# sandyz1000/deep-insight-face

Measured on AMD Instinct MI355X. Metric: faces/sec embedding+match (112x112, 512-d), higher is better.
Workload: dtype f32; 1 GPU; configs[3]: IResNet-100 embed, batch=512/GPU (4096 on 8 GPUs), 1M gallery row-sharded; arch=iresnet100, head=v2, batch_per_gpu=512, global_batch=512, gallery_rows=1000000, gallery_rows_per_gpu=1000000, emd=512, metric=cosine, parallelism=dp1 + gallery row-shard

## Files before the change

### deep-insight-face_amd/csrc/conv_winograd.hpp

```cpp
namespace wino {
constexpr int BN = 64;
constexpr int KC = 16;
constexpr int64_t MIN_TILES = 64 * 49;
constexpr int WIDE_MAX_HW = 112;
constexpr int64_t WIDE_MIN_IMAGES = 128;
constexpr int ODD_MAX_HW = 16;
constexpr int64_t ODD_MIN_TILES = 128 * 16;
}

template <int TT_, int CPW_, int MIN_BLOCKS_, bool EARLY_REQ_>
struct WinoW {
  static constexpr int TT = TT_;
  static constexpr int CPW = CPW_;
  static constexpr int MIN_BLOCKS = MIN_BLOCKS_;
  static constexpr bool EARLY_REQ = EARLY_REQ_;
  static constexpr bool ODD = false;
  static constexpr bool YSUB = false;
  static constexpr int MF = TT / 32;
  static constexpr int NT = 16 / CPW * 64;
  static constexpr int STAGE = 16 * TT * wino::KC;
  static constexpr int LDS_BYTES = 2 * STAGE * 4;
  static_assert(NT / 8 == TT && CPW % 2 == 0, "one loader thread per (tile, channel pair)");
};

template <bool ODD_, bool YSUB_>
struct WinoX : WinoW<32, 4, 2, true> {
  static constexpr bool ODD = ODD_;
  static constexpr bool YSUB = YSUB_;
  static_assert(!(ODD_ && YSUB_), "y_sub is admitted on even maps only");
};

__device__ __forceinline__ void wino_bt4(float x0, float x1, float x2, float x3, float& o0, float& o1, float& o2, float& o3) {
  o0 = x0 - x2;
  o1 = x1 + x2;
  o2 = x2 - x1;
  o3 = x1 - x3;
}

__device__ __forceinline__ void wino_input_transform(const float (&d)[16], float (&v)[16]) {
  float t[16];
#pragma unroll
  for (int c = 0; c < 4; ++c) wino_bt4(d[c], d[4 + c], d[8 + c], d[12 + c], t[c], t[4 + c], t[8 + c], t[12 + c]);
#pragma unroll
  for (int r = 0; r < 4; ++r) wino_bt4(t[4 * r], t[4 * r + 1], t[4 * r + 2], t[4 * r + 3], v[4 * r], v[4 * r + 1], v[4 * r + 2], v[4 * r + 3]);
}

template <bool TRACE>
__device__ __forceinline__ unsigned long long wino_stamp() {
  if constexpr (TRACE) return __builtin_amdgcn_s_memrealtime();
  return 0ull;
}
__device__ __forceinline__ void wino_trace_write(const ConvArgs& a, unsigned long long c0, const unsigned long long (&ts)[5]) {
  unsigned long long* t = a.trace + (size_t)blockIdx.x * 8;
  t[0] = ts[2] - ts[1];
  t[1] = ts[1] - ts[0];
  t[2] = ts[3] - ts[2];
  t[3] = ts[4] - ts[3];
  t[4] = (unsigned long long)__builtin_amdgcn_s_getreg((31 << 11) | 4) | ((unsigned long long)__builtin_amdgcn_s_getreg((31 << 11) | 20) << 32);
  t[5] = ts[0];
  t[6] = ts[4];
  t[7] = 3 | ((__builtin_amdgcn_s_memtime() - c0) << 8);
}

template <class S, bool TRACE>
__global__ __launch_bounds__(S::NT, S::MIN_BLOCKS) void conv_wino_kernel(const ConvArgs a, int blocks_m, int nblocks) {
  constexpr int TT = S::TT, CPW = S::CPW, MF = S::MF, KC = wino::KC;
  extern __shared__ __attribute__((aligned(16))) float wino_smem[];
  const int b = xcd_remap((int)blockIdx.x, nblocks);
  const int nt = b / blocks_m, mt = b - nt * blocks_m;
  const int tid = threadIdx.x, lane = tid & 63;
  const int wave = (S::ODD || S::YSUB) ? __builtin_amdgcn_readfirstlane(tid >> 6) : tid >> 6;
  const int tw = S::ODD ? (a.W + 1) >> 1 : a.W >> 1, tpi = (S::ODD ? (a.H + 1) >> 1 : a.H >> 1) * tw, ntiles = a.N * tpi;
  const int KS = a.Cin / KC;
  unsigned long long ts[5];
  ts[0] = wino_stamp<TRACE>();
  const unsigned long long tr_c0 = TRACE ? __builtin_amdgcn_s_memtime() : 0ull;

  const int ltile = tid >> 3, cp = tid & 7;
  const int g = mt * TT + ltile;
  const bool tile_ok = g < ntiles;
  int pix0 = 0;
  unsigned vmask = 0;
  if (tile_ok) {
    const int img = g / tpi, rem = g - img * tpi, ty = rem / tw, tx = rem - ty * tw;
    pix0 = (img * a.H + 2 * ty) * a.W + 2 * tx;
#pragma unroll
    for (int p = 0; p < 16; ++p) {
      const int iy = 2 * ty - 1 + (p >> 2), ix = 2 * tx - 1 + (p & 3);
      if (iy >= 0 && iy < a.H && ix >= 0 && ix < a.W) vmask |= 1u << p;
    }
  }
  const int row_b = a.W * a.Cin * 4, pix_b = a.Cin * 4;
  const int lbase = (pix0 - a.W - 1) * pix_b + cp * 8;
  const __amdgpu_buffer_rsrc_t xrs = make_rsrc(a.x, (uint32_t)a.N * (uint32_t)(a.H * a.W) * (uint32_t)pix_b);
  auto dload = [&](int ks, f32x2 (&d)[16]) {
#pragma unroll
    for (int p = 0; p < 16; ++p) {
      const uint32_t off = ((vmask >> p) & 1u) ? (uint32_t)(lbase + (p >> 2) * row_b + (p & 3) * pix_b + ks * (KC * 4)) : OOB;
      d[p] = __builtin_bit_cast(f32x2, __builtin_amdgcn_raw_buffer_load_b64(xrs, off, 0, 0));
    }
  };
  const int vdst = ltile * KC + (((cp >> 1) ^ ((ltile >> 2) & 3)) << 2) + (cp & 1) * 2;
  auto vstore = [&](float* buf, const f32x2 (&d)[16]) {
    float d0[16], d1[16], v0[16], v1[16];
#pragma unroll
    for (int p = 0; p < 16; ++p) {
      d0[p] = d[p][0];
      d1[p] = d[p][1];
    }
    wino_input_transform(d0, v0);
    wino_input_transform(d1, v1);
#pragma unroll
    for (int c = 0; c < 16; ++c) *reinterpret_cast<f32x2*>(buf + c * (TT * KC) + vdst) = f32x2{v0[c], v1[c]};
  };

  const int h = lane >> 5, r32 = lane & 31, sw = (r32 >> 2) & 3;
  const int tiles_n = a.Cout / wino::BN;
  const __amdgpu_buffer_rsrc_t wrs = make_rsrc(a.w_wino, a.w_wino_bytes);
  const uint32_t boff0 = (uint32_t)((CPW * wave * tiles_n + nt) * KS) * 4096u + (uint32_t)lane * 16u;
  const uint32_t bstep = (uint32_t)(tiles_n * KS) * 4096u;
  f32x4 bw[2][2][2];
  auto bload = [&](int j, int ks) {
#pragma unroll
    for (int nf = 0; nf < 2; ++nf)
#pragma unroll
      for (int q = 0; q < 2; ++q)
        bw[j & 1][nf][q] = buf_load4(wrs, boff0 + (uint32_t)j * bstep + (uint32_t)ks * 4096u + (uint32_t)(nf * 2 + q) * 1024u);
  };
  int aoff[2];
#pragma unroll
  for (int q = 0; q < 2; ++q) aoff[q] = r32 * KC + (((2 * h + q) ^ sw) << 2);
  f32x4 av[2][MF][2];
  auto aread = [&](const float* buf, int j) {
#pragma unroll
    for (int mf = 0; mf < MF; ++mf)
#pragma unroll
      for (int q = 0; q < 2; ++q)
        av[j & 1][mf][q] = *reinterpret_cast<const f32x4*>(buf + (CPW * wave + j) * (TT * KC) + mf * 32 * KC + aoff[q]);
  };
  f32x16 acc[CPW][MF][2];
#pragma unroll
  for (int j = 0; j < CPW; ++j)
#pragma unroll
    for (int mf = 0; mf < MF; ++mf)
#pragma unroll
      for (int nf = 0; nf < 2; ++nf)
#pragma unroll
        for (int r = 0; r < 16; ++r) acc[j][mf][nf][r] = 0.f;
  auto mfma = [&](int j) {
#pragma unroll
    for (int q = 0; q < 2; ++q)
#pragma unroll
      for (int t = 0; t < 4; ++t)
#pragma unroll
        for (int mf = 0; mf < MF; ++mf)
#pragma unroll
          for (int nf = 0; nf < 2; ++nf)
            acc[j][mf][nf] = __builtin_amdgcn_mfma_f32_32x32x2f32(av[j & 1][mf][q][t], bw[j & 1][nf][q][t], acc[j][mf][nf], 0, 0, 0);
  };

  {
    f32x2 d[16];
    dload(0, d);
    bload(0, 0);
    bload(1, 0);
    vstore(wino_smem, d);
    lds_barrier();
    ts[1] = wino_stamp<TRACE>();
    auto step = [&](int ks, auto last) {
      const float* cur = wino_smem + (ks & 1) * S::STAGE;
      float* nxt = wino_smem + ((ks + 1) & 1) * S::STAGE;
      aread(cur, 0);
      aread(cur, 1);
#pragma unroll
      for (int j = 0; j < CPW; ++j) {
        mfma(j);
        __builtin_amdgcn_sched_barrier(0);
        if (j + 2 < CPW) {
          aread(cur, j + 2);
          bload(j + 2, ks);
        } else if (!last.value) {
          bload(j + 2 - CPW, ks + 1);
        }
        if (!last.value && j == CPW / 2 - 1) dload(ks + 1, d);
        __builtin_amdgcn_sched_barrier(0);
      }
      if (!last.value) vstore(nxt, d);
      lds_barrier();
    };
    for (int ks = 0; ks + 1 < KS; ++ks) step(ks, std::false_type{});
    step(KS - 1, std::true_type{});
  }
  ts[2] = wino_stamp<TRACE>();

  const int c4 = cp * 4;
  const uint32_t bytes = (uint32_t)a.M * (uint32_t)a.Cout * 4u;
  const __amdgpu_buffer_rsrc_t y_rsrc = make_rsrc(a.y, a.y ? (S::YSUB ? (uint32_t)ntiles * (uint32_t)a.Cout * 4u : bytes) : 0u);
  const __amdgpu_buffer_rsrc_t y2_rsrc = make_rsrc(a.y2, a.y2 ? bytes : 0u);
  const __amdgpu_buffer_rsrc_t res_rsrc = make_rsrc(a.res, a.res ? bytes : 0u);
  const bool has_res = a.res != nullptr;
  const int act = a.act, act2 = a.act2;
#pragma unroll
  for (int nf = 0; nf < 2; ++nf) {
    const int c = nt * wino::BN + nf * 32 + c4;
    f32x4 sc, sh, al, sc2, sh2, al2, rv[4];
    uint32_t voff[4];
    if constexpr (S::EARLY_REQ) {
      sc = load4_or(a.scale, c, 1.f), sh = load4_or(a.shift, c, 0.f), al = load4_or(a.alpha, c, 0.f);
      sc2 = load4_or(a.scale2, c, 1.f), sh2 = load4_or(a.shift2, c, 0.f), al2 = load4_or(a.alpha2, c, 0.f);
#pragma unroll
      for (int p = 0; p < 4; ++p) {
        const int pix = pix0 + (p >> 1) * a.W + (p & 1);
        if constexpr (S::ODD)
          voff[p] = ((vmask >> (5 + 4 * (p >> 1) + (p & 1))) & 1u) ? ((uint32_t)pix * (uint32_t)a.Cout + (uint32_t)c) * 4u : OOB;
        else
          voff[p] = tile_ok ? ((uint32_t)pix * (uint32_t)a.Cout + (uint32_t)c) * 4u : OOB;
        rv[p] = has_res ? buf_load4(res_rsrc, voff[p]) : f32x4{0.f, 0.f, 0.f, 0.f};
      }
      __builtin_amdgcn_sched_barrier(0);
    }
#pragma unroll
    for (int j = 0; j < CPW; ++j)
#pragma unroll
      for (int mf = 0; mf < MF; ++mf)
#pragma unroll
        for (int r = 0; r < 16; ++r)
          wino_smem[(CPW * wave + j) * (TT * 32) + (mf * 32 + frag_row(lane, r)) * 32 + r32] = acc[j][mf][nf][r];
    lds_barrier();
    f32x4 m[16];
#pragma unroll
    for (int k = 0; k < 16; ++k) m[k] = *reinterpret_cast<const f32x4*>(wino_smem + k * (TT * 32) + ltile * 32 + c4);
    f32x4 yv[4];
    {
      f32x4 s0[4], s1[4];
#pragma unroll
      for (int jj = 0; jj < 4; ++jj) {
        s0[jj] = m[jj] + m[4 + jj] + m[8 + jj];
        s1[jj] = m[4 + jj] - m[8 + jj] - m[12 + jj];
      }
      yv[0] = s0[0] + s0[1] + s0[2];
      yv[1] = s0[1] - s0[2] - s0[3];
      yv[2] = s1[0] + s1[1] + s1[2];
      yv[3] = s1[1] - s1[2] - s1[3];
    }
    if constexpr (!S::EARLY_REQ) {
      sc = load4_or(a.scale, c, 1.f), sh = load4_or(a.shift, c, 0.f), al = load4_or(a.alpha, c, 0.f);
      sc2 = load4_or(a.scale2, c, 1.f), sh2 = load4_or(a.shift2, c, 0.f), al2 = load4_or(a.alpha2, c, 0.f);
#pragma unroll
      for (int p = 0; p < 4; ++p) {
        const int pix = pix0 + (p >> 1) * a.W + (p & 1);
        if constexpr (S::ODD)
          voff[p] = ((vmask >> (5 + 4 * (p >> 1) + (p & 1))) & 1u) ? ((uint32_t)pix * (uint32_t)a.Cout + (uint32_t)c) * 4u : OOB;
        else
          voff[p] = tile_ok ? ((uint32_t)pix * (uint32_t)a.Cout + (uint32_t)c) * 4u : OOB;
        rv[p] = has_res ? buf_load4(res_rsrc, voff[p]) : f32x4{0.f, 0.f, 0.f, 0.f};
      }
    }
#pragma unroll
    for (int p = 0; p < 4; ++p) {
      f32x4 v, v2;
      epilogue4(yv[p], sc, sh, al, act, has_res, rv[p], sc2, sh2, al2, act2, v, v2);
      if constexpr (S::YSUB) {
        if (p == 0) __builtin_amdgcn_raw_buffer_store_b128(__builtin_bit_cast(u32x4, v), y_rsrc, tile_ok ? ((uint32_t)g * (uint32_t)a.Cout + (uint32_t)c) * 4u : OOB, 0, 0);
      } else {
        __builtin_amdgcn_raw_buffer_store_b128(__builtin_bit_cast(u32x4, v), y_rsrc, voff[p], 0, 0);
      }
      __builtin_amdgcn_raw_buffer_store_b128(__builtin_bit_cast(u32x4, v2), y2_rsrc, voff[p], 0, 0);
    }
    lds_barrier();
    ts[3 + nf] = wino_stamp<TRACE>();
  }
  if constexpr (TRACE)
    if (tid == 0) wino_trace_write(a, tr_c0, ts);
}

static int wino_applies(const ConvArgs& a) {
  if (!a.w_wino || a.wino_level < 1 || a.KH != 3 || a.KW != 3 || a.stride != 1 || a.pad_t != 1 || a.pad_l != 1) return 0;
  if (a.Ho != a.H || a.Wo != a.W) return 0;
  const bool odd = (a.H & 1) || (a.W & 1), rest = odd || a.y_sub;
  const bool wide = a.H > 16 || a.W > 16;
  if (rest && (a.wino_level < 2 || (odd && (a.y_sub || a.H > wino::ODD_MAX_HW || a.W > wino::ODD_MAX_HW || a.H < 3 || a.W < 3)))) return 0;
  if (wide && (a.wino_level < 2 || a.H > wino::WIDE_MAX_HW || a.W > wino::WIDE_MAX_HW)) return 0;
  if (a.Cin % 32 != 0 || a.Cout % wino::BN != 0 || a.pre_scale) return 0;
  if (!(a.y_H == a.Ho && a.y_W == a.Wo && a.y_oy == 0 && a.y_ox == 0 && a.y_ld == a.Cout && a.y_coff == 0)) return 0;
  if (a.res && (a.res_stride != 1 || a.res_H != a.Ho || a.res_W != a.Wo)) return 0;
  if ((int64_t)a.M * a.Cout * 4 >= 0x7fffffffLL || (int64_t)a.M * a.Cin * 4 >= 0x7fffffffLL) return 0;
  if ((int64_t)16 * a.Cin * a.Cout * 4 > (int64_t)a.w_wino_bytes) return 0;
  const int64_t tpi = (int64_t)((a.H + 1) / 2) * ((a.W + 1) / 2);
  if (rest) return a.N >= wino::WIDE_MIN_IMAGES && (!odd || a.N * tpi >= wino::ODD_MIN_TILES) ? 3 : 0;
  if (wide) return a.N * tpi >= wino::WIDE_MIN_IMAGES * tpi ? 2 : 0;
  return a.N * tpi >= wino::MIN_TILES ? 1 : 0;
}

template <class S>
static int launch_wino(const ConvArgs& a, hipStream_t st, const char* name) {
  const auto kern = a.trace ? conv_wino_kernel<S, true> : conv_wino_kernel<S, false>;
  if (allow_dynamic_lds(reinterpret_cast<const void*>(kern), S::LDS_BYTES)) return -1;
  const int64_t ntiles = S::ODD ? (int64_t)a.N * ((a.H + 1) / 2) * ((a.W + 1) / 2) : (int64_t)a.N * (a.H / 2) * (a.W / 2);
  const int blocks_m = (int)((ntiles + S::TT - 1) / S::TT), tiles_n = a.Cout / wino::BN;
  const int64_t nblocks = (int64_t)blocks_m * tiles_n;
  if (nblocks >= 0x7fffffffLL) return set_error("conv: too many tiles");
  hipLaunchKernelGGL(kern, dim3((unsigned)nblocks), dim3(S::NT), S::LDS_BYTES, st, a, blocks_m, (int)nblocks);
  DIF_HIP(hipGetLastError());
  g_last_kernel = name;
  return 0;
}

static int launch_conv_wino(const ConvArgs& a, hipStream_t st) {
  if (a.wino_level >= 2 && !(a.dbg & 16777216)) return launch_wino<WinoW<32, 4, 2, true>>(a, st, "conv_wino_kernel<F(2x2,3x3),32 tiles x 64>");
  return launch_wino<WinoW<64, 2, 1, false>>(a, st, "conv_wino_kernel<F(2x2,3x3),64 tiles x 64>");
}

static int launch_conv_winow(const ConvArgs& a, hipStream_t st) {
  if (a.dbg & 65536) return launch_wino<WinoW<64, 2, 2, true>>(a, st, "conv_winow_kernel<F(2x2,3x3),64 tiles x 64>");
  return launch_wino<WinoW<32, 4, 2, true>>(a, st, "conv_winow_kernel<F(2x2,3x3),32 tiles x 64>");
}

static int launch_conv_winox(const ConvArgs& a, hipStream_t st) {
  if (a.y_sub) return launch_wino<WinoX<false, true>>(a, st, "conv_winox_kernel<F(2x2,3x3),32 tiles x 64,ysub>");
  return launch_wino<WinoX<true, false>>(a, st, "conv_winox_kernel<F(2x2,3x3),32 tiles x 64,odd>");
}
```

### deep-insight-face_amd/csrc/net.hip

```cpp
#include "net.hpp"

#include <math.h>
#include <stdio.h>
#include <stdlib.h>
#include <string.h>

#include <algorithm>
#include <map>

#include "../../include/dif.h"
#include "dif_internal.hpp"
#include "gemm_core.hpp"

namespace dif {

static const float EPS_RESNET = 1.001e-5f;
static const float EPS_KERAS = 1e-3f;
static const float EPS_IRESNET = 1e-5f;

Net::~Net() { release_device(); }

void Net::release_device() {
  for (Lane& L : lanes) {
    if (L.stream) (void)hipStreamDestroy(L.stream);
// ... 1266 lines not shown
      a.pad_l = op.pad_l;
      a.Kpad = op.Kpad;
      a.k_order = op.k_order;
      a.M = n * yd.H * yd.W;
      a.act = op.act;
      a.act2 = op.act2;
      a.y_sub = op.y_sub;
      if (op.res >= 0) {
        a.res_H = tensors[op.res].H;
        a.res_W = tensors[op.res].W;
        a.res_stride = op.res_stride;
      } else {
        a.res_H = yd.H;
        a.res_W = yd.W;
        a.res_stride = 1;
      }
      {
        const TensorDesc& vd = tensors[op.y >= 0 ? op.y : op.y2];
        if (vd.parent >= 0) {
          const TensorDesc& pd = tensors[vd.parent];
          a.y_ld = pd.C;
          a.y_coff = vd.coff;
          a.y_H = pd.H;
          a.y_W = pd.W;
          a.y_oy = vd.oy;
          a.y_ox = vd.ox;
        } else {
          a.y_ld = op.Cout;
          a.y_coff = 0;
          a.y_H = yd.H;
          a.y_W = yd.W;
          a.y_oy = a.y_ox = 0;
        }
      }
      a.sk_slab = L.sk_slab;
      a.sk_flag = L.sk_flag;
      a.sk_max_blocks = lanes_active ? L.sk_max_blocks : sk_max_blocks;
      a.sk_epoch = ++L.sk_epoch;
      a.sk_spin_limit = sk_spin_limit;
      a.use_pipe = use_pipe;
      a.off = conv_off;
      a.dbg = conv_dbg;
      a.lanes = lanes_active ? (int)lanes.size() : 1;
      a.bdp_mode = use_bdp == 2 ? 2 : ((use_bdp == 0 || lane_split) ? 1 : 0);
      a.trace = trace_buf ? trace_buf + trace_off[&op - ops.data()] * 8 : nullptr;
      if (op.d_w_raw && op.stem_mfma && use_stem) {
        if (stem_mfma_run(a.x, op.d_w_raw, a.scale, a.shift, a.alpha, a.scale2, a.shift2, a.alpha2, a.y, a.y2, n, a.H, a.W,
                          a.Ho, a.Wo, a.KH, a.stride, a.act, a.act2, a.y_sub, st))
          return -1;
        break;
      }
      if (op.d_w_raw && use_stem) {
        if (stem3x3_run(a.x, op.d_w_raw, a.scale, a.shift, a.alpha, a.scale2, a.shift2, a.alpha2, a.y, a.y2, n, a.H, a.W, a.Cout,
                        a.act, a.act2, st))
          return -1;
        break;
      }
      if (conv_run(a, st)) return -1;
      op.ran_kernel = conv_last_kernel();
      break;
    }
    case OP_MAXPOOL: {
      const TensorDesc& xd = tensors[op.x];
      const TensorDesc& yd = tensors[op.y];
      PoolArgs a;
      memset(&a, 0, sizeof(a));
      a.x = ptr(op.x);
      a.y = ptr(op.y);
      a.y2 = ptr(op.y2);
      a.scale2 = op.d_scale2;
      a.shift2 = op.d_shift2;
      a.N = n;
      a.H = xd.H;
      a.W = xd.W;
      a.C = xd.C;
      a.Ho = yd.H;
      a.Wo = yd.W;
      a.k = op.KH;
      a.stride = op.stride;
      a.pad_t = op.pad_t;
      a.pad_l = op.pad_l;
      a.zero_pad = op.zero_pad;
      a.act2 = op.act2;
      a.mode = op.pool_mode;
      if (yd.parent >= 0) {
        const TensorDesc& pd = tensors[yd.parent];
        a.y_ld = pd.C;
        a.y_coff = yd.coff;
        a.y_H = pd.H;
        a.y_W = pd.W;
        a.y_oy = yd.oy;
        a.y_ox = yd.ox;
      } else {
        a.y_ld = yd.C;
        a.y_coff = 0;
        a.y_H = yd.H;
        a.y_W = yd.W;
        a.y_oy = a.y_ox = 0;
      }
      if (maxpool_run(a, st)) return -1;
      break;
    }
    case OP_GDCTAIL: {
      const TensorDesc& xd = tensors[op.x];
      if (gdc_tail_run(ptr(op.x), op.d_w, op.d_scale, op.d_shift, op.d_w_pw, op.d_w_dense, ptr(op.y), n, xd.H * xd.W,
                       op.Cout, 1e-12f, L.tail_ws, st))
        return -1;
      op.ran_kernel = n <= 2 && op.Cout % 32 == 0 ? "gdc_tail_a_kernel+gdc_tail_b_kernel" : "gdc_tail_kernel";
      break;
    }
    case OP_DWFULL: {
      const TensorDesc& xd = tensors[op.x];
      if (dwfull_run(ptr(op.x), op.d_w, op.d_scale, op.d_shift, ptr(op.y), n, xd.H * xd.W, xd.C, st)) return -1;
      break;
    }
    case OP_DWCONV: {
      const TensorDesc& xd = tensors[op.x];
      const TensorDesc& yd = tensors[op.y];
      if (dwconv_run(ptr(op.x), op.d_w, op.d_scale, op.d_shift, ptr(op.y), n, xd.H, xd.W, xd.C, op.KH, op.stride, op.pad_t,
                     op.pad_l, yd.H, yd.W, op.act, st))
        return -1;
      break;
    }
    case OP_LRN: {
      const TensorDesc& xd = tensors[op.x];
      if (lrn_run(ptr(op.x), ptr(op.y), (int64_t)n * xd.H * xd.W, xd.C, 5, 1.f, 1e-4f, 0.75f, st)) return -1;
      break;
    }
    case OP_UPSAMPLE: {
      const TensorDesc& xd = tensors[op.x];
      const TensorDesc& yd = tensors[op.y];
      const int ld = yd.parent >= 0 ? tensors[yd.parent].C : yd.C;
      if (upsample2_run(ptr(op.x), ptr(op.y), n, xd.H, xd.W, xd.C, ld, yd.coff, st)) return -1;
      break;
    }
    case OP_COPY: {
      const TensorDesc& xd = tensors[op.x];
      const TensorDesc& yd = tensors[op.y];
      const int ld = yd.parent >= 0 ? tensors[yd.parent].C : yd.C;
      if (copy_to_view_run(ptr(op.x), ptr(op.y), (int64_t)n * xd.H * xd.W, xd.C, ld, yd.coff, st)) return -1;
      break;
    }
    case OP_ZERO: {
      const TensorDesc& yd = tensors[op.y];
      DIF_HIP(hipMemsetAsync(ptr(op.y), 0, (size_t)n * yd.elems() * sizeof(float), st));
      break;
    }
    case OP_L2NORM:
      if (l2norm_run(ptr(op.x), ptr(op.y), n, op.Cout, 1e-12f, st)) return -1;
      break;
  }
  return 0;
}

int Net::embed(const void* xin, int n, int layout, int dtype, float* out, hipStream_t st, float* op_ms) {
  if (!finalized) return set_error("dif_net_embed: call dif_net_finalize first");
  if (n < 0 || n > max_batch) return set_error("dif_net_embed: batch %d outside [0, max_batch=%d]", n, max_batch);
  if (n == 0) return 0;
  if (!xin || !out) return set_error("dif_net_embed: null pointer");
  if (layout != DIF_LAYOUT_NHWC && layout != DIF_LAYOUT_NCHW) return set_error("dif_net_embed: bad layout %d", layout);
  if (dtype != DIF_DTYPE_F32 && dtype != DIF_DTYPE_U8) return set_error("dif_net_embed: bad dtype %d", dtype);

  const int nl = (int)lanes.size();
  lanes_active = !(op_ms || nl == 1 || n < lane_min_images());
  lanes[0].out_n = n;
  lanes[0].out_start = 0;
  if (!lanes_active) {
    std::vector<hipEvent_t> ev;
    if (op_ms) {
      ev.resize(ops.size() + 1);
      for (auto& e : ev) DIF_HIP(hipEventCreate(&e));
      DIF_HIP(hipEventRecord(ev[0], st));
    }
    for (size_t i = 0; i < ops.size(); ++i) {
      if (run_op(ops[i], lanes[0], xin, n, layout, dtype, out, st)) return -1;
      if (op_ms) DIF_HIP(hipEventRecord(ev[i + 1], st));
    }
    if (op_ms) {
      DIF_HIP(hipStreamSynchronize(st));
      for (size_t i = 0; i < ops.size(); ++i) DIF_HIP(hipEventElapsedTime(&op_ms[i], ev[i], ev[i + 1]));
      for (auto& e : ev) (void)hipEventDestroy(e);
    }
    return 0;
  }

  const size_t in_bytes = (size_t)in_h * in_w * 3 * (dtype == DIF_DTYPE_U8 ? 1 : 4);
  std::vector<int> start(nl + 1, 0);
  for (int l = 0; l < nl; ++l) {
    int c = n / nl + (l < n % nl ? 1 : 0);
    if (l > 0 && c > lanes[l].cap) c = lanes[l].cap;
    start[l + 1] = start[l] + c;
  }
  const int l_first = lanes[0].stream ? 0 : 1;
  DIF_HIP(hipEventRecord(ev_start, st));
  for (int l = l_first; l < nl; ++l) DIF_HIP(hipStreamWaitEvent(lanes[l].stream, ev_start, 0));
  for (size_t i = 0; i < ops.size(); ++i) {
    for (int l = 0; l < nl; ++l) {
      const int c = start[l + 1] - start[l];
      if (c == 0) continue;
      hipStream_t ls = lanes[l].stream ? lanes[l].stream : st;
      lanes[l].out_n = n;
      lanes[l].out_start = start[l];
      if (run_op(ops[i], lanes[l], static_cast<const char*>(xin) + (size_t)start[l] * in_bytes, c, layout, dtype, out, ls))
        return -1;
    }
  }
  for (int l = l_first; l < nl; ++l) {
    DIF_HIP(hipEventRecord(lanes[l].done, lanes[l].stream));
    DIF_HIP(hipStreamWaitEvent(st, lanes[l].done, 0));
  }
  return 0;
}

int Net::embed_clock(const void* xin, int n, int layout, int dtype, float* out, hipStream_t st, double* ghz) {
  if (!finalized) return set_error("dif_net_embed_clock: call dif_net_finalize first");
  if (!ghz) return set_error("dif_net_embed_clock: null output");
  if (n < 1 || n > max_batch) return set_error("dif_net_embed_clock: batch %d outside [1, max_batch=%d]", n, max_batch);
  trace_off.assign(ops.size(), 0);
  size_t total = 0;
  for (size_t i = 0; i < ops.size(); ++i) {
    trace_off[i] = total;
    if (ops[i].kind != OP_CONV) continue;
    const TensorDesc& yd = tensors[ops[i].y >= 0 && !ops[i].y_sub ? ops[i].y : ops[i].y2];
    const size_t tiles = (((size_t)n * yd.H * yd.W + 63) / 64) * (((size_t)ops[i].Cout + 63) / 64);
    total += tiles > (size_t)sk_max_blocks ? tiles : (size_t)sk_max_blocks;
  }
  unsigned long long* d = nullptr;
  DIF_HIP(hipMalloc(&d, total * 8 * sizeof(unsigned long long)));
  DIF_HIP(hipMemsetAsync(d, 0, total * 8 * sizeof(unsigned long long), st));
  trace_buf = d;
  int rc = 0;
  lanes_active = false;
  lanes[0].out_n = n;
  lanes[0].out_start = 0;
  for (size_t i = 0; i < ops.size() && !rc; ++i) rc = run_op(ops[i], lanes[0], xin, n, layout, dtype, out, st);
  trace_buf = nullptr;
  std::vector<unsigned long long> h;
  if (!rc) {
    h.resize(total * 8);
    if (hipStreamSynchronize(st) != hipSuccess || hipMemcpy(h.data(), d, h.size() * sizeof(unsigned long long), hipMemcpyDeviceToHost) != hipSuccess)
      rc = set_error("dif_net_embed_clock: reading the records failed");
  }
  (void)hipFree(d);
  if (rc) return rc;
  if (conv_dbg & 256) {
    for (size_t i = 0; i < ops.size(); ++i) {
      if (ops[i].kind != OP_CONV) continue;
      const size_t end = i + 1 < ops.size() ? trace_off[i + 1] : total;
      unsigned long long t_lo = ~0ull, t_hi = 0;
      double life = 0, mn = 1e30, mx = 0, m = 0, f = 0, e = 0, steps = 0, tiles = 0;
      double p_set = 0, p_pro = 0, p_steps = 0, p_hand = 0, p_tiles = 0;
      double w_e0 = 0, w_e1 = 0;
      std::map<unsigned long long, std::vector<const unsigned long long*>> w_cu;
      int nb = 0;
      for (size_t b = trace_off[i]; b < end; ++b) {
        const unsigned long long* t = &h[b * 8];
        if ((t[7] & 0xff) == 0 || t[6] <= t[5]) continue;
        ++nb;
        t_lo = t[5] < t_lo ? t[5] : t_lo;
        t_hi = t[6] > t_hi ? t[6] : t_hi;
        const double l = (double)(t[6] - t[5]);
        life += l;
        mn = l < mn ? l : mn;
        mx = l > mx ? l : mx;
        if ((t[7] & 0xff) == 2) {
          p_set += (double)t[0];
          p_pro += (double)t[1];
          p_steps += (double)t[2];
          p_hand += (double)t[3];
          p_tiles += (double)t[4];
        }
        if ((t[7] & 0xff) == 1) {
          m += (double)t[0];
          f += (double)t[1];
          e += (double)t[2];
          steps += (double)t[3];
          tiles += (double)t[4];
        }
        if ((t[7] & 0xff) == 3) {
          m += (double)t[0];
          f += (double)t[1];
          e += (double)(t[2] + t[3]);
          w_e0 += (double)t[2];
          w_e1 += (double)t[3];
          tiles += 1;
          w_cu[((t[4] >> 32) & 0xf) << 16 | (t[4] & 0xff00)].push_back(t);
        }
      }
      if (nb)
        fprintf(stderr, "trace %-22s blocks %5d span %7.1f us | life mean %7.1f min %7.1f max %7.1f | main %6.1f fix %6.1f epi %6.1f us/block | "
                        "steps/block %.1f tiles/block %.2f\n", ops[i].name.c_str(), nb, (double)(t_hi - t_lo) / 100.0, life / nb / 100.0,
                mn / 100.0, mx / 100.0, m / nb / 100.0, f / nb / 100.0, e / nb / 100.0, steps / nb, tiles / nb);
      if (nb && !w_cu.empty()) {
        double ph = 0, lag = 0;
        int pairs = 0;
        for (auto& kv : w_cu)
          for (const unsigned long long* u : kv.second)
            for (const unsigned long long* v : kv.second)
              if (v != u && v[5] <= u[5] && u[5] < v[6] && (v[5] < u[5] || v < u)) {
                ph += (double)(u[5] - v[5]) / (double)(v[6] - v[5]);
                lag += (double)(u[5] - v[5]);
                ++pairs;
              }
        fprintf(stderr, "      winograd: epilogue halves %.1f + %.1f us/block | %zu CUs, %.2f blocks/CU | blocks starting beside a resident one: %d, "
                        "%.1f us = %.2f of its life after it\n", w_e0 / nb / 100.0, w_e1 / nb / 100.0, w_cu.size(), (double)nb / w_cu.size(), pairs,
                pairs ? lag / pairs / 100.0 : 0.0, pairs ? ph / pairs : 0.0);
      }
      if (nb && p_tiles > 0)
        fprintf(stderr, "      pipelined: %.2f tiles/block | per tile: set-up %.2f prologue %.2f K-steps %.2f hand-over %.2f us\n", p_tiles / nb,
                p_set / p_tiles / 100.0, p_pro / p_tiles / 100.0, p_steps / p_tiles / 100.0, p_hand / p_tiles / 100.0);
    }
  }
  if (conv_dbg & 512) {
    for (size_t i = 0; i < ops.size(); ++i) {
      if (ops[i].kind != OP_CONV) continue;
      const size_t end = i + 1 < ops.size() ? trace_off[i + 1] : total;
      std::map<unsigned, std::vector<double>> by_xcd, by_cu;
      unsigned long long t_lo = ~0ull;
      for (size_t b = trace_off[i]; b < end; ++b)
        if ((h[b * 8 + 7] & 0xff) == 1 && h[b * 8 + 4] && h[b * 8 + 5] < t_lo) t_lo = h[b * 8 + 5];
      int nb = 0;
      for (size_t b = trace_off[i]; b < end; ++b) {
        const unsigned long long* t = &h[b * 8];
        if ((t[7] & 0xff) != 1 || !t[4] || t[6] <= t[5]) continue;
        ++nb;
        const unsigned hw = (unsigned)t[4], xcc = (unsigned)(t[4] >> 32) & 0xf;
        const unsigned cu = (xcc << 16) | (hw & 0xff00);
        for (auto* mp : {&by_xcd[xcc], &by_cu[cu]}) {
          if (mp->empty()) mp->assign(5, 0.0);
          (*mp)[0] += 1;
          (*mp)[1] += (double)(t[6] - t[5]);
          (*mp)[2] += (double)(t[7] >> 8);
          (*mp)[3] = std::max((*mp)[3], (double)(t[6] - t_lo));
          (*mp)[4] += (double)(t[5] - t_lo);
        }
      }
      if (!nb) continue;
      fprintf(stderr, "place %-20s blocks %d on %zu CUs |", ops[i].name.c_str(), nb, by_cu.size());
      for (auto& kv : by_xcd)
        fprintf(stderr, " xcd%u: %d blk life %.0f us end %.0f us %.2f GHz |", kv.first, (int)kv.second[0], kv.second[1] / kv.second[0] / 100.0,
                kv.second[3] / 100.0, kv.second[2] / (kv.second[1] * 10.0));
      std::map<int, std::vector<double>> hist;
      for (auto& kv : by_cu) {
        auto& hrec = hist[(int)kv.second[0]];
        if (hrec.empty()) hrec.assign(4, 0.0);
        hrec[0] += 1;
        hrec[1] += kv.second[1] / kv.second[0];
        hrec[2] += kv.second[3];
        hrec[3] += kv.second[4] / kv.second[0];
      }
      for (auto& kv : hist)
        fprintf(stderr, " %d/CU: %d CUs life %.0f start %.0f end %.0f us |", kv.first, (int)kv.second[0], kv.second[1] / kv.second[0] / 100.0,
                kv.second[3] / kv.second[0] / 100.0, kv.second[2] / kv.second[0] / 100.0);
      double rl[8] = {0}, rn[8] = {0}, wl[16] = {0}, wn[16] = {0};
      for (size_t b = trace_off[i]; b < end; ++b) {
        const unsigned long long* t = &h[b * 8];
        if ((t[7] & 0xff) != 1 || !t[4] || t[6] <= t[5]) continue;
        const size_t r = std::min<size_t>((b - trace_off[i]) / by_cu.size(), 7);
        rl[r] += (double)(t[6] - t[5]);
        rn[r] += 1;
        wl[t[4] & 0xf] += (double)(t[6] - t[5]);
        wn[t[4] & 0xf] += 1;
      }
      for (int r = 0; r < 8; ++r)
        if (rn[r] > 0) fprintf(stderr, " round%d: %.0f us (%d) |", r, rl[r] / rn[r] / 100.0, (int)rn[r]);
      for (int r = 0; r < 16; ++r)
        if (wn[r] > 0) fprintf(stderr, " slot%d: %.0f us (%d) |", r, wl[r] / wn[r] / 100.0, (int)wn[r]);
      fprintf(stderr, "\n");
    }
  }
  double cyc = 0, ticks = 0;
  for (size_t b = 0; b < total; ++b) {
    const unsigned long long* t = &h[b * 8];
    const unsigned kind = (unsigned)(t[7] & 0xff);
    if ((kind == 1 || kind == 2) && t[6] > t[5]) {
      cyc += (double)(t[7] >> 8);
      ticks += (double)(t[6] - t[5]);
    }
  }
  *ghz = ticks > 0 ? cyc / (ticks * 10.0) : 0.0;
  return 0;
}

}
```

Before: 8853 faces/s.

## Fold Winograd output rows in registers and issue residual loads under last K-step

For the CPW=4 Winograd config, each wave now owns one column of the 4x4 transform grid. It performs the first stage of the output transform in registers, stages only two planes per nf to LDS, and finishes both channel halves in a single pass with one barrier. The old code staged all sixteen planes per half with two barriers. Residual loads are also issued during the final K-step so their latency hides behind MFMAs. This costs extra registers for the prefetched residuals and changes the weight and LDS indexing, which could lower occupancy.

```diff
diff --git a/deep-insight-face_amd/csrc/conv_winograd.hpp b/deep-insight-face_amd/csrc/conv_winograd.hpp
--- a/deep-insight-face_amd/csrc/conv_winograd.hpp
+++ b/deep-insight-face_amd/csrc/conv_winograd.hpp
@@ -7,6 +7,10 @@
 constexpr int ODD_MAX_HW = 16;
 constexpr int64_t ODD_MIN_TILES = 128 * 16;
 }
+
+#ifndef DIF_WINO_RES_UNDER_K
+#define DIF_WINO_RES_UNDER_K 1
+#endif
 
 template <int TT_, int CPW_, int MIN_BLOCKS_, bool EARLY_REQ_>
 struct WinoW {
@@ -20,7 +24,12 @@
   static constexpr int NT = 16 / CPW * 64;
   static constexpr int STAGE = 16 * TT * wino::KC;
   static constexpr int LDS_BYTES = 2 * STAGE * 4;
+  static constexpr bool ONE_PASS = CPW_ == 4;
+  static constexpr int COMP_W = ONE_PASS ? 1 : CPW_;
+  static constexpr int COMP_J = ONE_PASS ? 4 : 1;
+  static constexpr bool RES_UNDER_K = ONE_PASS && DIF_WINO_RES_UNDER_K;
   static_assert(NT / 8 == TT && CPW % 2 == 0, "one loader thread per (tile, channel pair)");
+  static_assert(!ONE_PASS || (TT == 32 && 8 * TT * wino::BN * 4 <= LDS_BYTES), "one pass: eight planes of 32 tiles x 64 channels");
 };
 
 template <bool ODD_, bool YSUB_>
@@ -117,8 +126,8 @@
   const int h = lane >> 5, r32 = lane & 31, sw = (r32 >> 2) & 3;
   const int tiles_n = a.Cout / wino::BN;
   const __amdgpu_buffer_rsrc_t wrs = make_rsrc(a.w_wino, a.w_wino_bytes);
-  const uint32_t boff0 = (uint32_t)((CPW * wave * tiles_n + nt) * KS) * 4096u + (uint32_t)lane * 16u;
-  const uint32_t bstep = (uint32_t)(tiles_n * KS) * 4096u;
+  const uint32_t boff0 = (uint32_t)((S::COMP_W * wave * tiles_n + nt) * KS) * 4096u + (uint32_t)lane * 16u;
+  const uint32_t bstep = (uint32_t)(S::COMP_J * tiles_n * KS) * 4096u;
   f32x4 bw[2][2][2];
   auto bload = [&](int j, int ks) {
 #pragma unroll
@@ -136,7 +145,7 @@
     for (int mf = 0; mf < MF; ++mf)
 #pragma unroll
       for (int q = 0; q < 2; ++q)
-        av[j & 1][mf][q] = *reinterpret_cast<const f32x4*>(buf + (CPW * wave + j) * (TT * KC) + mf * 32 * KC + aoff[q]);
+        av[j & 1][mf][q] = *reinterpret_cast<const f32x4*>(buf + (S::COMP_W * wave + S::COMP_J * j) * (TT * KC) + mf * 32 * KC + aoff[q]);
   };
   f32x16 acc[CPW][MF][2];
 #pragma unroll
@@ -157,6 +166,21 @@
 #pragma unroll
           for (int nf = 0; nf < 2; ++nf)
             acc[j][mf][nf] = __builtin_amdgcn_mfma_f32_32x32x2f32(av[j & 1][mf][q][t], bw[j & 1][nf][q][t], acc[j][mf][nf], 0, 0, 0);
+  };
+
+  uint32_t voff8[2][4];
+  f32x4 rv8[2][4];
+  auto res_request = [&]() {
+    const __amdgpu_buffer_rsrc_t res_rsrc = make_rsrc(a.res, a.res ? (uint32_t)a.M * (uint32_t)a.Cout * 4u : 0u);
+#pragma unroll
+    for (int nf = 0; nf < 2; ++nf)
+#pragma unroll
+      for (int p = 0; p < 4; ++p) {
+        const int pix = pix0 + (p >> 1) * a.W + (p & 1), c = nt * wino::BN + nf * 32 + cp * 4;
+        const uint32_t off_map = ((vmask >> (5 + 4 * (p >> 1) + (p & 1))) & 1u) - 1u;
+        voff8[nf][p] = (((uint32_t)pix * (uint32_t)a.Cout + (uint32_t)c) * 4u) | (off_map & OOB);
+        rv8[nf][p] = buf_load4(res_rsrc, voff8[nf][p]);
+      }
   };
 
   {
@@ -183,6 +207,7 @@
           bload(j + 2 - CPW, ks + 1);
         }
         if (!last.value && j == CPW / 2 - 1) dload(ks + 1, d);
+        if (last.value && S::RES_UNDER_K && j == CPW / 2 - 1) res_request();
         __builtin_amdgcn_sched_barrier(0);
       }
       if (!last.value) vstore(nxt, d);
@@ -200,75 +225,130 @@
   const __amdgpu_buffer_rsrc_t res_rsrc = make_rsrc(a.res, a.res ? bytes : 0u);
   const bool has_res = a.res != nullptr;
   const int act = a.act, act2 = a.act2;
-#pragma unroll
-  for (int nf = 0; nf < 2; ++nf) {
-    const int c = nt * wino::BN + nf * 32 + c4;
-    f32x4 sc, sh, al, sc2, sh2, al2, rv[4];
-    uint32_t voff[4];
-    if constexpr (S::EARLY_REQ) {
-      sc = load4_or(a.scale, c, 1.f), sh = load4_or(a.shift, c, 0.f), al = load4_or(a.alpha, c, 0.f);
-      sc2 = load4_or(a.scale2, c, 1.f), sh2 = load4_or(a.shift2, c, 0.f), al2 = load4_or(a.alpha2, c, 0.f);
-#pragma unroll
-      for (int p = 0; p < 4; ++p) {
-        const int pix = pix0 + (p >> 1) * a.W + (p & 1);
-        if constexpr (S::ODD)
-          voff[p] = ((vmask >> (5 + 4 * (p >> 1) + (p & 1))) & 1u) ? ((uint32_t)pix * (uint32_t)a.Cout + (uint32_t)c) * 4u : OOB;
-        else
-          voff[p] = tile_ok ? ((uint32_t)pix * (uint32_t)a.Cout + (uint32_t)c) * 4u : OOB;
-        rv[p] = has_res ? buf_load4(res_rsrc, voff[p]) : f32x4{0.f, 0.f, 0.f, 0.f};
-      }
-      __builtin_amdgcn_sched_barrier(0);
-    }
-#pragma unroll
-    for (int j = 0; j < CPW; ++j)
-#pragma unroll
-      for (int mf = 0; mf < MF; ++mf)
-#pragma unroll
-        for (int r = 0; r < 16; ++r)
-          wino_smem[(CPW * wave + j) * (TT * 32) + (mf * 32 + frag_row(lane, r)) * 32 + r32] = acc[j][mf][nf][r];
+  if constexpr (S::ONE_PASS) {
+    static_assert(MF == 1 && CPW == 4, "one row fragment, one grid column per wave");
+    if constexpr (!S::RES_UNDER_K) res_request();
+    f32x4 sc[2], sh[2], al[2], sc2[2], sh2[2], al2[2];
+#pragma unroll
+    for (int nf = 0; nf < 2; ++nf) {
+      const int c = nt * wino::BN + nf * 32 + c4;
+      sc[nf] = load4_or(a.scale, c, 1.f), sh[nf] = load4_or(a.shift, c, 0.f), al[nf] = load4_or(a.alpha, c, 0.f);
+      sc2[nf] = load4_or(a.scale2, c, 1.f), sh2[nf] = load4_or(a.shift2, c, 0.f), al2[nf] = load4_or(a.alpha2, c, 0.f);
+    }
+    __builtin_amdgcn_sched_barrier(0);
+#pragma unroll
+    for (int nf = 0; nf < 2; ++nf) {
+      acc[3][0][nf] = (acc[1][0][nf] - acc[2][0][nf]) - acc[3][0][nf];
+      acc[0][0][nf] = (acc[0][0][nf] + acc[1][0][nf]) + acc[2][0][nf];
+    }
+#pragma unroll
+    for (int nf = 0; nf < 2; ++nf)
+#pragma unroll
+      for (int r = 0; r < 16; ++r) {
+        wino_smem[(wave * 2 + nf) * (TT * 32) + frag_row(lane, r) * 32 + r32] = acc[0][0][nf][r];
+        wino_smem[((4 + wave) * 2 + nf) * (TT * 32) + frag_row(lane, r) * 32 + r32] = acc[3][0][nf][r];
+      }
     lds_barrier();
-    f32x4 m[16];
-#pragma unroll
-    for (int k = 0; k < 16; ++k) m[k] = *reinterpret_cast<const f32x4*>(wino_smem + k * (TT * 32) + ltile * 32 + c4);
-    f32x4 yv[4];
-    {
+    ts[3] = wino_stamp<TRACE>();
+#pragma unroll
+    for (int nf = 0; nf < 2; ++nf) {
       f32x4 s0[4], s1[4];
 #pragma unroll
       for (int jj = 0; jj < 4; ++jj) {
-        s0[jj] = m[jj] + m[4 + jj] + m[8 + jj];
-        s1[jj] = m[4 + jj] - m[8 + jj] - m[12 + jj];
-      }
+        s0[jj] = *reinterpret_cast<const f32x4*>(wino_smem + (jj * 2 + nf) * (TT * 32) + ltile * 32 + c4);
+        s1[jj] = *reinterpret_cast<const f32x4*>(wino_smem + ((4 + jj) * 2 + nf) * (TT * 32) + ltile * 32 + c4);
+      }
+      f32x4 yv[4];
       yv[0] = s0[0] + s0[1] + s0[2];
       yv[1] = s0[1] - s0[2] - s0[3];
       yv[2] = s1[0] + s1[1] + s1[2];
       yv[3] = s1[1] - s1[2] - s1[3];
-    }
-    if constexpr (!S::EARLY_REQ) {
-      sc = load4_or(a.scale, c, 1.f), sh = load4_or(a.shift, c, 0.f), al = load4_or(a.alpha, c, 0.f);
-      sc2 = load4_or(a.scale2, c, 1.f), sh2 = load4_or(a.shift2, c, 0.f), al2 = load4_or(a.alpha2, c, 0.f);
 #pragma unroll
       for (int p = 0; p < 4; ++p) {
-        const int pix = pix0 + (p >> 1) * a.W + (p & 1);
-        if constexpr (S::ODD)
-          voff[p] = ((vmask >> (5 + 4 * (p >> 1) + (p & 1))) & 1u) ? ((uint32_t)pix * (uint32_t)a.Cout + (uint32_t)c) * 4u : OOB;
-        else
-          voff[p] = tile_ok ? ((uint32_t)pix * (uint32_t)a.Cout + (uint32_t)c) * 4u : OOB;
-        rv[p] = has_res ? buf_load4(res_rsrc, voff[p]) : f32x4{0.f, 0.f, 0.f, 0.f};
-      }
-    }
-#pragma unroll
-    for (int p = 0; p < 4; ++p) {
-      f32x4 v, v2;
-      epilogue4(yv[p], sc, sh, al, act, has_res, rv[p], sc2, sh2, al2, act2, v, v2);
-      if constexpr (S::YSUB) {
-        if (p == 0) __builtin_amdgcn_raw_buffer_store_b128(__builtin_bit_cast(u32x4, v), y_rsrc, tile_ok ? ((uint32_t)g * (uint32_t)a.Cout + (uint32_t)c) * 4u : OOB, 0, 0);
-      } else {
-        __builtin_amdgcn_raw_buffer_store_b128(__builtin_bit_cast(u32x4, v), y_rsrc, voff[p], 0, 0);
-      }
-      __builtin_amdgcn_raw_buffer_store_b128(__builtin_bit_cast(u32x4, v2), y2_rsrc, voff[p], 0, 0);
-    }
-    lds_barrier();
-    ts[3 + nf] = wino_stamp<TRACE>();
+        f32x4 v, v2;
+        epilogue4(yv[p], sc[nf], sh[nf], al[nf], act, has_res, rv8[nf][p], sc2[nf], sh2[nf], al2[nf], act2, v, v2);
+        if constexpr (S::YSUB) {
+          if (p == 0)
+            __builtin_amdgcn_raw_buffer_store_b128(__builtin_bit_cast(u32x4, v), y_rsrc,
+                                                   tile_ok ? ((uint32_t)g * (uint32_t)a.Cout + (uint32_t)(nt * wino::BN + nf * 32 + c4)) * 4u : OOB, 0, 0);
+        } else {
+          __builtin_amdgcn_raw_buffer_store_b128(__builtin_bit_cast(u32x4, v), y_rsrc, voff8[nf][p], 0, 0);
+        }
+        __builtin_amdgcn_raw_buffer_store_b128(__builtin_bit_cast(u32x4, v2), y2_rsrc, voff8[nf][p], 0, 0);
+      }
+    }
+    ts[4] = wino_stamp<TRACE>();
+  } else {
+#pragma unroll
+    for (int nf = 0; nf < 2; ++nf) {
+      const int c = nt * wino::BN + nf * 32 + c4;
+      f32x4 sc, sh, al, sc2, sh2, al2, rv[4];
+      uint32_t voff[4];
+      if constexpr (S::EARLY_REQ) {
+        sc = load4_or(a.scale, c, 1.f), sh = load4_or(a.shift, c, 0.f), al = load4_or(a.alpha, c, 0.f);
+        sc2 = load4_or(a.scale2, c, 1.f), sh2 = load4_or(a.shift2, c, 0.f), al2 = load4_or(a.alpha2, c, 0.f);
+#pragma unroll
+        for (int p = 0; p < 4; ++p) {
+          const int pix = pix0 + (p >> 1) * a.W + (p & 1);
+          if constexpr (S::ODD)
+            voff[p] = ((vmask >> (5 + 4 * (p >> 1) + (p & 1))) & 1u) ? ((uint32_t)pix * (uint32_t)a.Cout + (uint32_t)c) * 4u : OOB;
+          else
+            voff[p] = tile_ok ? ((uint32_t)pix * (uint32_t)a.Cout + (uint32_t)c) * 4u : OOB;
+          rv[p] = has_res ? buf_load4(res_rsrc, voff[p]) : f32x4{0.f, 0.f, 0.f, 0.f};
+        }
+        __builtin_amdgcn_sched_barrier(0);
+      }
+#pragma unroll
+      for (int j = 0; j < CPW; ++j)
+#pragma unroll
+        for (int mf = 0; mf < MF; ++mf)
+#pragma unroll
+          for (int r = 0; r < 16; ++r)
+            wino_smem[(CPW * wave + j) * (TT * 32) + (mf * 32 + frag_row(lane, r)) * 32 + r32] = acc[j][mf][nf][r];
+      lds_barrier();
+      f32x4 m[16];
+#pragma unroll
+      for (int k = 0; k < 16; ++k) m[k] = *reinterpret_cast<const f32x4*>(wino_smem + k * (TT * 32) + ltile * 32 + c4);
+      f32x4 yv[4];
+      {
+        f32x4 s0[4], s1[4];
+#pragma unroll
+        for (int jj = 0; jj < 4; ++jj) {
+          s0[jj] = m[jj] + m[4 + jj] + m[8 + jj];
+          s1[jj] = m[4 + jj] - m[8 + jj] - m[12 + jj];
+        }
+        yv[0] = s0[0] + s0[1] + s0[2];
+        yv[1] = s0[1] - s0[2] - s0[3];
+        yv[2] = s1[0] + s1[1] + s1[2];
+        yv[3] = s1[1] - s1[2] - s1[3];
+      }
+      if constexpr (!S::EARLY_REQ) {
+        sc = load4_or(a.scale, c, 1.f), sh = load4_or(a.shift, c, 0.f), al = load4_or(a.alpha, c, 0.f);
+        sc2 = load4_or(a.scale2, c, 1.f), sh2 = load4_or(a.shift2, c, 0.f), al2 = load4_or(a.alpha2, c, 0.f);
+#pragma unroll
+        for (int p = 0; p < 4; ++p) {
+          const int pix = pix0 + (p >> 1) * a.W + (p & 1);
+          if constexpr (S::ODD)
+            voff[p] = ((vmask >> (5 + 4 * (p >> 1) + (p & 1))) & 1u) ? ((uint32_t)pix * (uint32_t)a.Cout + (uint32_t)c) * 4u : OOB;
+          else
+            voff[p] = tile_ok ? ((uint32_t)pix * (uint32_t)a.Cout + (uint32_t)c) * 4u : OOB;
+          rv[p] = has_res ? buf_load4(res_rsrc, voff[p]) : f32x4{0.f, 0.f, 0.f, 0.f};
+        }
+      }
+#pragma unroll
+      for (int p = 0; p < 4; ++p) {
+        f32x4 v, v2;
+        epilogue4(yv[p], sc, sh, al, act, has_res, rv[p], sc2, sh2, al2, act2, v, v2);
+        if constexpr (S::YSUB) {
+          if (p == 0) __builtin_amdgcn_raw_buffer_store_b128(__builtin_bit_cast(u32x4, v), y_rsrc, tile_ok ? ((uint32_t)g * (uint32_t)a.Cout + (uint32_t)c) * 4u : OOB, 0, 0);
+        } else {
+          __builtin_amdgcn_raw_buffer_store_b128(__builtin_bit_cast(u32x4, v), y_rsrc, voff[p], 0, 0);
+        }
+        __builtin_amdgcn_raw_buffer_store_b128(__builtin_bit_cast(u32x4, v2), y2_rsrc, voff[p], 0, 0);
+      }
+      lds_barrier();
+      ts[3 + nf] = wino_stamp<TRACE>();
+    }
   }
   if constexpr (TRACE)
     if (tid == 0) wino_trace_write(a, tr_c0, ts);
diff --git a/deep-insight-face_amd/csrc/net.hip b/deep-insight-face_amd/csrc/net.hip
--- a/deep-insight-face_amd/csrc/net.hip
+++ b/deep-insight-face_amd/csrc/net.hip
@@ -1592,7 +1592,7 @@
                 lag += (double)(u[5] - v[5]);
                 ++pairs;
               }
-        fprintf(stderr, "      winograd: epilogue halves %.1f + %.1f us/block | %zu CUs, %.2f blocks/CU | blocks starting beside a resident one: %d, "
+        fprintf(stderr, "      winograd: epilogue halves | stage + finish %.1f + %.1f us/block | %zu CUs, %.2f blocks/CU | blocks starting beside a resident one: %d, "
                         "%.1f us = %.2f of its life after it\n", w_e0 / nb / 100.0, w_e1 / nb / 100.0, w_cu.size(), (double)nb / w_cu.size(), pairs,
                 pairs ? lag / pairs / 100.0 : 0.0, pairs ? ph / pairs : 0.0);
       }
```

After: 8992 faces/s, median of 6. 1.02x the previous value.
